# yjh0410/YOLO-Nano

Measured on AMD Instinct MI355X. Metric: images/sec YOLO-Nano-1.0x 416x416 bs=32 inference (network + decode + NMS + host delivery), higher is better.
Workload: dtype f32 (split-f16 MFMA x3, fp32 accumulate); 1 GPU; YOLO-Nano-1.0x 416x416 bs=32/GPU fp32 inference, COCO 80-class head + NMS (BASELINE configs[1]); inputs resident in HBM, kept detections delivered to pinned host memory inside the timed region; global_batch=32, parallelism=image-sharded x1, no collective, rccl_ranks=1, launch_mode=eager, streams_per_gpu=4

## Files before the change

yolo-nano_amd/csrc/kernels_post.hip:

```cpp
#include "yn_device.h"
#include "yn_head_tile_map.h"
#include "yn_prep.h"

namespace ynk {

__device__ __forceinline__ float sigmoid_f(float v) { return 1.0f / (1.0f + expf(-v)); }
__device__ __forceinline__ float exp_le0(float x) { return __builtin_amdgcn_exp2f(x * 1.44269504088896340736f); }

__device__ __forceinline__ void cand_location(const GridInfo& g, int n, int& s, int& cell, int& a)
{
    s = (n >= g.off[2]) ? 2 : ((n >= g.off[1]) ? 1 : 0);
    const int local = n - g.off[s];
    cell = local / g.A;
    a = local - cell * g.A;
}

__device__ __forceinline__ float grid_window_norm(const GridInfo& g, float p, int k)
{
    return (p + (float)((k & 1) ? g.top : g.left)) / (float)g.side;
}

__device__ __forceinline__ void decode_one(const GridInfo& g, int s, int cell, int a, const float* t, float S, float* box, bool normalise)
{
    const int gy = cell / g.w[s], gx = cell - gy * g.w[s];
// ... 1700 lines not shown
    const int n = seg_count[(size_t)b * C + c];
    const int T = (n + 63) >> 6;
    const bool sliced = rank < sliced_ranks && T - 1 > YN_PRE_W;
    const int ZS = sliced ? min(YN_PRE_Z, (T - 1 + YN_PRE_W - 1) / YN_PRE_W) : 1;
    bool decide = false;
    if (sliced && seg_sparse && sweep_slots > 0 && large_list && nms_colmajor(n)) {
        const int32_t* ll = large_list + (size_t)b * (large_cap + 1);
        const int nl = ll[0] < sweep_slots ? ll[0] : sweep_slots;
        for (int k = 0; k < nl; ++k) decide |= ll[1 + k] == c;
    }
    const bool decider = decide && z == ZS;
    if (z >= ZS && !decider) return;
    if (n == 0) { if (threadIdx.x == 0) { seg_count2[(size_t)b * C + c] = 0; if (seg_sparse) seg_sparse[(size_t)b * C + c] = 0; } return; }
    const int off = seg_off[(size_t)b * C + c];
    const float4* sb = sbox + (size_t)b * N + off;
    const int32_t* ids = bucket + (size_t)b * N + off;
    const int tid = threadIdx.x, lane = tid & 63;
    const int wave = __builtin_amdgcn_readfirstlane((int)(tid >> 6));
    const size_t slot = (size_t)b * YN_PRE_RANKS + (rank < YN_PRE_RANKS ? rank : 0);
    u64* ticket = pre_sync + slot;
    u64* gs = pre_sync + YN_PRE_TICKETS + slot * pre_sync_words(N);
    if (decider) {
        const bool sp = sweep_spread_out(sb, n, L);
        if (tid == 0) __hip_atomic_store(&gs[0], sp ? 1ull : 0ull, __ATOMIC_RELAXED, __HIP_MEMORY_SCOPE_AGENT);
    } else {
        float4* cbox = L.cbox[wave];
        float* carea = L.carea[wave];
        float4 bx0 = make_float4(0.f, 0.f, 0.f, 0.f);
        if (lane < n) bx0 = sb[lane];
        {
            u64 part = 0;
            if (wave * 8 < n) part = tile_word_boxes<false>(bx0, bx0, n, 0, 0, thresh, cbox, carea, wave * 8, wave * 8 + 8);
            L.dpart[lane][wave] = (unsigned char)(part >> (8 * wave));
        }
        __syncthreads();
        if (wave == 0) {
            const u64 diag = *reinterpret_cast<const u64*>(L.dpart[lane]);
            const int cnt = min(64, n);
            u64 alive = cnt == 64 ? ~0ull : ((1ull << cnt) - 1ull);
            u64 work = __ballot(((alive >> lane) & 1ull) && (diag & alive));
            const unsigned dlo = (unsigned)(diag & 0xffffffffu), dhi = (unsigned)(diag >> 32);
            while (work) {
                const int i = __ffsll((long long)work) - 1;
                const unsigned lo_i = (unsigned)__builtin_amdgcn_readlane((int)dlo, i);
                const unsigned hi_i = (unsigned)__builtin_amdgcn_readlane((int)dhi, i);
                alive &= ~(((u64)hi_i << 32) | (u64)lo_i);
                work &= alive & ~(1ull << i);
            }
            if (((alive >> lane) & 1ull) && z == 0) keep[(size_t)b * N + ids[lane]] = 1;
            if (lane == 0) L.keepm = alive;
        }
        if (T == 1) {
            if (tid == 0) { seg_count2[(size_t)b * C + c] = 0; if (seg_sparse) seg_sparse[(size_t)b * C + c] = 0; }
            return;
        }
        __syncthreads();
        const u64 keepm = L.keepm;
        const float4 bx = bx0;
        float4 cb = make_float4(0.f, 0.f, 0.f, 0.f), cbn = cb;
        int ci = 1 + z * YN_PRE_W + wave;
        if (ci < T && ci * 64 + lane < n) cb = sb[ci * 64 + lane];
        for (; ci < T; ci += YN_PRE_W * ZS) {
            const int cn = ci + YN_PRE_W * ZS;
            cbn = make_float4(0.f, 0.f, 0.f, 0.f);
            if (cn < T && cn * 64 + lane < n) cbn = sb[cn * 64 + lane];
            u64 w = keepm ? tile_word_boxes<false>(bx, cb, n, 0, ci, thresh, cbox, carea) : 0ull;
            w = ((keepm >> lane) & 1ull) ? w : 0ull;
            unsigned lo = (unsigned)(w & 0xffffffffu), hi = (unsigned)(w >> 32);
#pragma unroll
            for (int o = 32; o >= 1; o >>= 1) { lo |= __shfl_xor(lo, o); hi |= __shfl_xor(hi, o); }
            const int cnt = min(64, n - ci * 64);
            const u64 valid = cnt == 64 ? ~0ull : ((1ull << cnt) - 1ull);
            const u64 sv = valid & ~(((u64)hi << 32) | (u64)lo);
            if (lane == 0) { if (sliced) __hip_atomic_store(&gs[ci], sv, __ATOMIC_RELAXED, __HIP_MEMORY_SCOPE_AGENT); else L.surv[ci] = sv; }
            cb = cbn;
        }
    }
    bool spread = false;
    if (sliced) {
        asm volatile("s_waitcnt vmcnt(0)" ::: "memory");
        __syncthreads();
        if (tid == 0) {
            const u64 t = __hip_atomic_fetch_add(ticket, 1ull, __ATOMIC_RELAXED, __HIP_MEMORY_SCOPE_AGENT);
            L.last = t == (u64)(ZS + (decide ? 1 : 0) - 1);
            if (L.last) __hip_atomic_store(ticket, 0ull, __ATOMIC_RELAXED, __HIP_MEMORY_SCOPE_AGENT);
        }
        __syncthreads();
        if (!L.last) return;
        for (int k = 1 + tid; k < T; k += NTH) L.surv[k] = __hip_atomic_load(&gs[k], __ATOMIC_RELAXED, __HIP_MEMORY_SCOPE_AGENT);
        if (decide) spread = __hip_atomic_load(&gs[0], __ATOMIC_RELAXED, __HIP_MEMORY_SCOPE_AGENT) != 0ull;
    }
    __syncthreads();
    const int Q = (T - 1 + NTH - 1) / NTH;
    int mine = 0;
    for (int q = 0; q < Q; ++q) { const int ci = 1 + tid * Q + q; if (ci < T) mine += __popcll(L.surv[ci]); }
    L.part[tid] = mine;
    __syncthreads();
    for (int o = 1; o < NTH; o <<= 1) {
        const int v = tid >= o ? L.part[tid - o] : 0;
        __syncthreads();
        L.part[tid] += v;
        __syncthreads();
    }
    int run = L.part[tid] - mine;
    for (int q = 0; q < Q; ++q) { const int ci = 1 + tid * Q + q; if (ci < T) { L.base[ci] = run; run += __popcll(L.surv[ci]); } }
    const int n2 = L.part[NTH - 1];
    if (tid == NTH - 1) {
        seg_count2[(size_t)b * C + c] = n2;
        if (seg_sparse) seg_sparse[(size_t)b * C + c] = (spread && nms_colmajor(n2) && n2 <= sweep_maxn) ? 1 : 0;
    }
    __syncthreads();
    for (int ci = 1 + wave; ci < T; ci += YN_PRE_W) {
        const u64 m = L.surv[ci];
        if ((m >> lane) & 1ull) {
            const int dst = L.base[ci] + __popcll(m & ((1ull << lane) - 1ull));
            sbox2[(size_t)b * N + off + dst] = sb[ci * 64 + lane];
            bucket2[(size_t)b * N + off + dst] = ids[ci * 64 + lane];
        }
    }
}

__global__ __launch_bounds__(1024) void nms_sweep_kernel(const float4* __restrict__ sbox, const int32_t* __restrict__ seg_count, const int32_t* __restrict__ seg_off,
                                                         const int32_t* __restrict__ tile_off, int N, int C, float thresh, u64* __restrict__ M, size_t m_stride,
                                                         const int32_t* __restrict__ large_list, int large_cap, const int32_t* __restrict__ seg_sparse, int maxn)
{
    extern __shared__ __attribute__((aligned(16))) float4 sw_box[];
    __shared__ int start[YN_SWEEP_BINS + 2];
    __shared__ int irr[YN_SWEEP_IRR];
    __shared__ int wide[YN_SWEEP_WIDE];
    __shared__ int n_wide;
    __shared__ unsigned xlo_u, xhi_u;
    __shared__ int n_irr;
    const int b = blockIdx.x;
    const int32_t* ll = large_list + (size_t)b * (large_cap + 1);
    if ((int)blockIdx.z >= ll[0]) return;
    const int c = ll[1 + blockIdx.z];
    const int n = seg_count[(size_t)b * C + c];
    if (!nms_colmajor(n) || n > maxn || !seg_sparse[(size_t)b * C + c]) return;
    const float4* sb = sbox + (size_t)b * N + seg_off[(size_t)b * C + c];
    int* sw_order = reinterpret_cast<int*>(sw_box + n);
    const int tid = threadIdx.x, lane = tid & 63, wave = tid >> 6;
    for (int i = tid; i < YN_SWEEP_BINS + 2; i += 1024) start[i] = 0;
    if (tid == 0) { xlo_u = 0xffffffffu; xhi_u = 0u; n_irr = 0; n_wide = 0; }
    __syncthreads();
    {
        unsigned mn = 0xffffffffu, mx = 0u;
        for (int i = tid; i < n; i += 1024) {
            const float4 bx = sb[i];
            sw_box[i] = bx;
            if (sweep_regular(bx)) { mn = min(mn, order_bits(bx.x)); mx = max(mx, order_bits(bx.z)); }
            else { const int k = atomicAdd(&n_irr, 1); if (k < YN_SWEEP_IRR) irr[k] = i; }
        }
#pragma unroll
        for (int o = 32; o >= 1; o >>= 1) { mn = min(mn, (unsigned)__shfl_xor((int)mn, o)); mx = max(mx, (unsigned)__shfl_xor((int)mx, o)); }
        if (lane == 0) { atomicMin(&xlo_u, mn); atomicMax(&xhi_u, mx); }
    }
    __syncthreads();
    const int nirr = n_irr;
    const SweepBins bins(xlo_u, xhi_u);
    auto bin_of = [&](float x) { return bins.of(x); };
    for (int i = tid; i < n; i += 1024) {
        const float4 bx = sw_box[i];
        if (sweep_regular(bx)) atomicAdd(&start[bin_of(bx.x) + 2], 1);
    }
    __syncthreads();
    if (wave == 0) {
        int mine = 0;
        for (int q = 0; q < YN_SWEEP_BINS / 64; ++q) mine += start[2 + lane * (YN_SWEEP_BINS / 64) + q];
        int incl = mine;
#pragma unroll
        for (int o = 1; o < 64; o <<= 1) { const int v = __shfl_up(incl, o); if (lane >= o) incl += v; }
        int run = incl - mine;
        for (int q = 0; q < YN_SWEEP_BINS / 64; ++q) { const int k = 2 + lane * (YN_SWEEP_BINS / 64) + q; const int cnt = start[k]; start[k] = run; run += cnt; }
    }
    __syncthreads();
    for (int i = tid; i < n; i += 1024) {
        const float4 bx = sw_box[i];
        if (sweep_regular(bx)) sw_order[atomicAdd(&start[bin_of(bx.x) + 2], 1)] = i;
    }
    __syncthreads();
    u64* Ms = M + (size_t)b * m_stride + (size_t)tile_off[(size_t)b * (C + 1) + c] * 64;
    const float c_hi = thresh * 1.00001f, c_lo = thresh * 0.99999f;
    auto test = [&](int i, int j, const float4 bi, float ai, const float4 bj) {
        const float aj = (bj.z - bj.x) * (bj.w - bj.y);
        const float w = vmax_raw(1e-28f, vmin_raw(bi.z, bj.z) - vmax_raw(bi.x, bj.x));
        const float h = vmax_raw(1e-28f, vmin_raw(bi.w, bj.w) - vmax_raw(bi.y, bj.y));
        const float inter = w * h;
        const float un = (ai + aj) - inter;
        const float hi = un * c_hi, lo = un * c_lo;
        bool hit;
        if (lo > 1e-30f && inter < lo) return;
        if (lo > 1e-30f && inter > hi) hit = true;
        else hit = suppressed(bi, ai, bj, aj, thresh, 0);
        if (hit) {
            const int r = i < j ? i : j, t = i < j ? j : i;
            atomicOr(Ms + ctile_off(r >> 6, t >> 6) + (r & 63), 1ull << (t & 63));
        }
    };
    const int kz = blockIdx.y, KZ = gridDim.y;
    const int grp = tid >> 4, gl = tid & 15;
    for (int i = kz + KZ * grp; i < n; i += 64 * KZ) {
        const float4 bi = sw_box[i];
        if (!sweep_regular(bi)) continue;
        const float ai = (bi.z - bi.x) * (bi.w - bi.y);
        const int q0 = bin_of(bi.x), q1 = bin_of(bi.z);
        const int p0 = start[q0 + 1], pm = start[q0 + 2], p1 = start[q1 + 2];
        if (p1 - p0 > YN_SWEEP_WIDE_VISITS) {
            int k = 0;
            if (gl == 0) k = atomicAdd(&n_wide, 1);
            k = __shfl(k, 0, 16);
            if (k < YN_SWEEP_WIDE) { if (gl == 0) wide[k] = i; continue; }
        }
        for (int p = p0 + gl; p < p1; p += 16) {
            const int j = sw_order[p];
            if (p < pm ? j > i : true) test(i, j, bi, ai, sw_box[j]);
        }
    }
    __syncthreads();
    {
        const int nw = n_wide < YN_SWEEP_WIDE ? n_wide : YN_SWEEP_WIDE;
        for (int k = 0; k < nw; ++k) {
            const int i = wide[k];
            const float4 bi = sw_box[i];
            const float ai = (bi.z - bi.x) * (bi.w - bi.y);
            const int q0 = bin_of(bi.x), q1 = bin_of(bi.z);
            const int p0 = start[q0 + 1], pm = start[q0 + 2], p1 = start[q1 + 2];
            for (int p = p0 + tid; p < p1; p += 1024) {
                const int j = sw_order[p];
                if (p < pm ? j > i : true) test(i, j, bi, ai, sw_box[j]);
            }
        }
    }
    for (int k = 0; k < nirr; ++k) {
        const int i = irr[k];
        const float4 bi = sw_box[i];
        const float ai = (bi.z - bi.x) * (bi.w - bi.y);
        for (int j = kz + KZ * tid; j < n; j += 1024 * KZ) {
            if (j == i) continue;
            const float4 bj = sw_box[j];
            if (sweep_regular(bj) || j > i) test(i, j, bi, ai, bj);
        }
    }
}

__global__ __launch_bounds__(64) void nms_tile_off_kernel(const int32_t* __restrict__ seg_count2, int C, int32_t* __restrict__ tile_off2, const int32_t* __restrict__ seg_sparse,
                                                          int32_t* __restrict__ work_off)
{
    const int b = blockIdx.x, lane = threadIdx.x;
    int tiles = 0, wtiles = 0;
    for (int c0 = 0; c0 < C; c0 += 64) {
        const int c = c0 + lane;
        int t = 0, w = 0;
        if (c < C) {
            const int T = (seg_count2[(size_t)b * C + c] + 63) >> 6;
            t = T * (T + 1) / 2;
            w = (seg_sparse && seg_sparse[(size_t)b * C + c]) ? 0 : t;
        }
        int ti = t, wi = w;
#pragma unroll
        for (int o = 1; o < 64; o <<= 1) { const int a = __shfl_up(ti, o), d = __shfl_up(wi, o); if (lane >= o) { ti += a; wi += d; } }
        if (c < C) {
            tile_off2[(size_t)b * (C + 1) + c] = tiles + ti - t;
            if (work_off) work_off[(size_t)b * (C + 1) + c] = wtiles + wi - w;
        }
        tiles += __shfl(ti, 63);
        wtiles += __shfl(wi, 63);
    }
    if (lane == 0) {
        tile_off2[(size_t)b * (C + 1) + C] = tiles;
        if (work_off) work_off[(size_t)b * (C + 1) + C] = wtiles;
    }
}

__global__ __launch_bounds__(1024) void single_sort_kernel(const float* __restrict__ dets, const float* __restrict__ scores, int n,
                                                           int32_t* __restrict__ ids, float4* __restrict__ sbox, u64* __restrict__ gscratch)
{
    extern __shared__ __attribute__((aligned(16))) unsigned char sort_lds[];
    if (gscratch) sort_segment<false>(dets, scores, ids, false, n, nms_pow2(n), gscratch, sbox);
    else sort_segment<true>(dets, scores, ids, false, n, nms_pow2(n), reinterpret_cast<u64*>(sort_lds), sbox);
}

template <bool DIOU>
__global__ __launch_bounds__(64) void single_matrix_kernel(const float4* __restrict__ sbox, int n, float thresh, u64* __restrict__ M)
{
    __shared__ float4 cbox[64];
    __shared__ float carea[64];
    const int T = (n + 63) >> 6;
    const int total = T * (T + 1) / 2;
    for (int t = blockIdx.x; t < total; t += gridDim.x) {
        int rem = t, ri = 0;
        while (rem >= T - ri) { rem -= T - ri; ++ri; }
        matrix_tile<DIOU>(sbox, n, T, ri, ri + rem, thresh, M, cbox, carea);
    }
}

__global__ __launch_bounds__(256) void single_resolve_kernel(const int32_t* __restrict__ ids, int n, const u64* __restrict__ M,
                                                              int32_t* __restrict__ pick_list, int32_t* __restrict__ count)
{
    __shared__ ResolveLds L;
    const int picked = n > 0 ? resolve_segment<2>(ids, n, M, nullptr, pick_list, L) : 0;
    if (threadIdx.x == 0) *count = picked;
}

__global__ __launch_bounds__(1024) void compact_kernel(const float* __restrict__ boxes, const float* __restrict__ scores,
                                                        const int32_t* __restrict__ cls, const int32_t* __restrict__ keep, int N,
                                                        float* __restrict__ out_boxes, float* __restrict__ out_scores,
                                                        int32_t* __restrict__ out_cls, int32_t* __restrict__ out_index,
                                                        int32_t* __restrict__ count, const unsigned* __restrict__ ovf, unsigned* __restrict__ ovf_host)
{
    constexpr int IT = 32;
    __shared__ int wave_sums[IT][16];
    __shared__ int part[8];
    __shared__ int base, total_next;
    const int b = blockIdx.x;
    const int lane = threadIdx.x & 63, wave = threadIdx.x >> 6;
    if (threadIdx.x == 0) base = 0;
    __syncthreads();
    for (int n0 = 0; n0 < N; n0 += IT * 1024) {
        int kf[IT];
#pragma unroll
        for (int it = 0; it < IT; ++it) {
            const int n = n0 + it * 1024 + threadIdx.x;
            kf[it] = keep[(size_t)b * N + (n < N ? n : N - 1)];
        }
        unsigned flags = 0;
        int before[IT];
#pragma unroll
        for (int it = 0; it < IT; ++it) {
            const int n = n0 + it * 1024 + threadIdx.x;
            const int f = (n < N && kf[it]) ? 1 : 0;
            const unsigned long long bal = __ballot(f);
            before[it] = __popcll(bal & ((1ull << lane) - 1ull));
            if (lane == 0) wave_sums[it][wave] = __popcll(bal);
            flags |= (unsigned)f << it;
        }
        __syncthreads();
        int v = 0, incl = 0;
        if (threadIdx.x < IT * 16) {
            v = (&wave_sums[0][0])[threadIdx.x];
            incl = v;
#pragma unroll
            for (int o = 1; o < 64; o <<= 1) { const int t2 = __shfl_up(incl, o); if (lane >= o) incl += t2; }
            if (lane == 63) part[wave] = incl;
        }
        __syncthreads();
        if (threadIdx.x < IT * 16) {
            int add = 0;
#pragma unroll
            for (int w = 0; w < 8; ++w) add += (w < wave) ? part[w] : 0;
            (&wave_sums[0][0])[threadIdx.x] = base + add + incl - v;
            if (threadIdx.x == IT * 16 - 1) total_next = base + add + incl;
        }
        __syncthreads();
#pragma unroll
        for (int g8 = 0; g8 < IT; g8 += 8) {
            float4 bx[8]; float sc[8]; int cl[8];
#pragma unroll
            for (int k = 0; k < 8; ++k) {
                const int it = g8 + k;
                const int n = n0 + it * 1024 + threadIdx.x;
                const size_t src = (size_t)b * N + (((flags >> it) & 1u) ? n : 0);
                bx[k] = *reinterpret_cast<const float4*>(boxes + src * 4);
                sc[k] = scores[src];
                cl[k] = cls[src];
            }
#pragma unroll
            for (int k = 0; k < 8; ++k) {
                const int it = g8 + k;
                if ((flags >> it) & 1u) {
                    const int n = n0 + it * 1024 + threadIdx.x;
                    const size_t dst = (size_t)b * N + wave_sums[it][wave] + before[it];
                    *reinterpret_cast<float4*>(out_boxes + dst * 4) = bx[k];
                    out_scores[dst] = sc[k];
                    out_cls[dst] = cl[k];
                    if (out_index) out_index[dst] = n;
                }
            }
        }
        __syncthreads();
        if (threadIdx.x == 0) base = total_next;
        __syncthreads();
    }
    if (threadIdx.x == 0) {
        const bool flagged = ovf && *ovf;
        count[b] = flagged ? -1 - base : base;
        if (flagged && ovf_host) __hip_atomic_store(ovf_host, 1u, __ATOMIC_RELAXED, __HIP_MEMORY_SCOPE_SYSTEM);
    }
}

int nms_max_segment() { return 64 * YN_RESOLVE_MAX_T; }

__global__ __launch_bounds__(256) void pack_kernel(const float* __restrict__ boxes, const float* __restrict__ scores, const int32_t* __restrict__ cls,
                                                   const int32_t* __restrict__ count, int B, int N, float* __restrict__ rec, int32_t* __restrict__ offsets)
{
    __shared__ int base_s, total_s;
    const int b = blockIdx.x;
    if (threadIdx.x < 64) {
        int mine = 0, all = 0;
        int bad = 0;
        for (int i = threadIdx.x; i < B; i += 64) { int c = count[i]; if (c < 0) { bad = 1; c = -1 - c; } all += c; if (i < b) mine += c; }
        for (int o = 32; o > 0; o >>= 1) { mine += __shfl_xor(mine, o); all += __shfl_xor(all, o); bad |= __shfl_xor(bad, o); }
        if (threadIdx.x == 0) { base_s = mine; total_s = bad ? -1 - all : all; }
    }
    __syncthreads();
    const int base = base_s, k = count[b] < 0 ? -1 - count[b] : count[b];
    if (threadIdx.x == 0) { offsets[b] = base; if (b == 0) offsets[B] = total_s; }
    for (int i = threadIdx.x; i < k; i += 256) {
        const size_t src = (size_t)b * N + i;
        const float4 bx = *reinterpret_cast<const float4*>(boxes + src * 4);
        float* r = rec + (size_t)(base + i) * 6;
        *reinterpret_cast<float2*>(r) = make_float2(bx.x, bx.y);
        *reinterpret_cast<float2*>(r + 2) = make_float2(bx.z, bx.w);
        *reinterpret_cast<float2*>(r + 4) = make_float2(scores[src], (float)cls[src]);
    }
}

void launch_pack(const float* boxes, const float* scores, const int32_t* cls, const int32_t* count, int B, int N, float* rec, int32_t* offsets, hipStream_t s)
{
    hipLaunchKernelGGL(pack_kernel, dim3(B), dim3(256), 0, s, boxes, scores, cls, count, B, N, rec, offsets);
}

size_t nms_pre_sync_words(int B, int N) { return YN_PRE_TICKETS + (size_t)B * YN_PRE_RANKS * pre_sync_words(N); }
size_t nms_matrix_words_per_image(int N, int C)
{
    const size_t Tsum = (size_t)(N + 63) / 64 + C;
    return 64 * (Tsum * (Tsum + 1) / 2);
}

static void set_sort_attr()
{
    static unsigned long long done = 0;
    if (!attr_pending(done)) return;
    (void)hipFuncSetAttribute(reinterpret_cast<const void*>(sort_kernel), hipFuncAttributeMaxDynamicSharedMemorySize, YN_SORT_LARGE * 8);
    (void)hipFuncSetAttribute(reinterpret_cast<const void*>(single_sort_kernel), hipFuncAttributeMaxDynamicSharedMemorySize, YN_SORT_LARGE * 8);
}

const int32_t* launch_nms_bucket_sort(const float* boxes, const float* scores, const int32_t* cls, int B, int N, int C, const NmsWork& wk,
                                      hipStream_t s, const NmsHook* hook, NmsPlan& rec)
{
    set_sort_attr();
    const int large_cap = wk.large_cap;
    auto mark = [&](const char* k) { if (hook && hook->fn) hook->fn(hook->ctx, k); };
    float4* sbox = reinterpret_cast<float4*>(wk.sbox);
    u64* M = reinterpret_cast<u64*>(wk.matrix);
    constexpr int few_n = 16384;
    const bool few = (long)B * C <= 256 && N <= few_n;
    const int32_t* seg_order = wk.seg_order;
    rec.few = few;
    if (few && wk.ctr) {
        seg_order = nullptr;
        rec.fused = 1;
        static unsigned long long attr_bs = 0;
        if (attr_pending(attr_bs)) (void)hipFuncSetAttribute(reinterpret_cast<const void*>(bucket_sort_kernel), hipFuncAttributeMaxDynamicSharedMemorySize, YN_SORT_LARGE * 8);
        mark("bucket_sort_kernel");
        hipLaunchKernelGGL(bucket_sort_kernel, dim3(C, B), dim3(1024), YN_SORT_LARGE * 8, s, boxes, scores, cls, N, C, wk.seg_count, wk.seg_off, wk.tile_off, wk.bucket,
                           wk.keep, sbox, M, wk.matrix_stride, wk.ctr);
    } else {
        mark("bucket_kernel");
        hipLaunchKernelGGL(bucket_kernel, dim3(B), dim3(1024), 2 * C * sizeof(int32_t), s, cls, N, C, wk.seg_count, wk.seg_off, wk.tile_off, wk.bucket, wk.keep,
                           wk.large_list, large_cap, YN_SORT_SMALL, wk.seg_order);
        const bool chunks = !few && wk.large_list && (size_t)N <= wk.matrix_stride;
        rec.chunks = chunks;
        mark(chunks ? "sort_chunk_kernel" : "sort_kernel");
        if (few) {
            hipLaunchKernelGGL(sort_kernel, dim3(B, C), dim3(1024), YN_SORT_LARGE * 8, s, boxes, scores, wk.seg_count, wk.seg_off, wk.bucket, sbox,
                               N, C, 0, YN_SORT_LARGE, (u64*)nullptr, (size_t)0, (const int32_t*)nullptr, 0, (const int32_t*)wk.seg_order);
        } else if (chunks) {
            const int slots = N > YN_SORT_SMALL ? nms_chunk_slots(N, large_cap) : 0;
            hipLaunchKernelGGL(sort_chunk_kernel, dim3(B, C + slots), dim3(256), YN_SORT_SMALL * 8, s, boxes, scores, wk.seg_count, wk.seg_off, wk.bucket, sbox,
                               N, C, (const int32_t*)wk.seg_order, (const int32_t*)wk.large_list, large_cap, M, wk.matrix_stride);
            if (N > YN_SORT_SMALL) {
                mark("sort_merge_kernel");
                rec.merge = 1;
                hipLaunchKernelGGL(sort_merge_kernel, dim3((N + 255) / 256, B), dim3(256), 0, s, boxes, wk.seg_count, wk.seg_off, wk.bucket, sbox,
                                   N, C, (const int32_t*)wk.large_list, large_cap, (const u64*)M, wk.matrix_stride);
            }
        } else {
            hipLaunchKernelGGL(sort_kernel, dim3(B, C), dim3(256), YN_SORT_SMALL * 8, s, boxes, scores, wk.seg_count, wk.seg_off, wk.bucket, sbox,
                               N, C, 0, YN_SORT_SMALL, (u64*)nullptr, (size_t)0, (const int32_t*)nullptr, 0, (const int32_t*)wk.seg_order);
            if (N > YN_SORT_SMALL)
                hipLaunchKernelGGL(sort_kernel, dim3(large_cap, B), dim3(1024), YN_SORT_LARGE * 8, s, boxes, scores, wk.seg_count, wk.seg_off, wk.bucket, sbox,
                                   N, C, YN_SORT_SMALL, YN_SORT_LARGE, (u64*)nullptr, (size_t)0, (const int32_t*)wk.large_list, large_cap, (const int32_t*)nullptr);
        }
        if (N > YN_SORT_LARGE && !chunks)
            hipLaunchKernelGGL(sort_kernel, dim3(large_cap, B), dim3(1024), 0, s, boxes, scores, wk.seg_count, wk.seg_off, wk.bucket, sbox,
                               N, C, YN_SORT_LARGE, 1 << 30, M, wk.matrix_stride, (const int32_t*)wk.large_list, large_cap, (const int32_t*)nullptr);
    }
    return seg_order;
}

void launch_nms_compact(const float* boxes, const float* scores, const int32_t* cls, int B, int N, const NmsWork& wk,
                        float* out_boxes, float* out_scores, int32_t* out_cls, int32_t* out_index, int32_t* count, hipStream_t s)
{
    hipLaunchKernelGGL(compact_kernel, dim3(B), dim3(1024), 0, s, boxes, scores, cls, wk.keep, N, out_boxes, out_scores, out_cls, out_index, count, wk.ovf, wk.ovf_host);
}

void launch_nms_pipeline(const float* boxes, const float* scores, const int32_t* cls, int B, int N, int C,
                         float nms_thresh, int diou, const NmsWork& wk,
                         float* out_boxes, float* out_scores, int32_t* out_cls, int32_t* out_index, int32_t* count,
                         hipStream_t s, const NmsHook* hook, NmsPlan* plan)
{
    NmsPlan rec{};
    rec.B = B; rec.N = N; rec.C = C; rec.diou = diou != 0;
    const int large_cap = wk.large_cap;
    auto mark = [&](const char* k) { if (hook && hook->fn) hook->fn(hook->ctx, k); };
    float4* sbox = reinterpret_cast<float4*>(wk.sbox);
    u64* M = reinterpret_cast<u64*>(wk.matrix);
    const int32_t* seg_order = launch_nms_bucket_sort(boxes, scores, cls, B, N, C, wk, s, hook, rec);
    const bool few = rec.few != 0;
    const int32_t* m_count = wk.seg_count;
    const int32_t* m_toff = wk.tile_off;
    const int32_t* m_ids = wk.bucket;
    const float4* m_box = sbox;
    const int prefilter_env = wk.prefilter;
    bool sweep = false;
    int sweep_maxn = 0, sweep_slots = 0;
    if (!diou && wk.sbox2 && (prefilter_env == 2 || (prefilter_env == 1 && B >= 4))) {
        mark("nms_prefilter_kernel");
        sweep = wk.sweep && !few && wk.seg_sparse && wk.work_off && wk.large_list && large_cap > 0 && N > YN_SORT_SMALL && nms_thresh >= 1e-6f;
        sweep_maxn = N <= 16384 ? YN_SWEEP_MAXN / 2 : YN_SWEEP_MAXN;
        sweep_slots = large_cap < 4 ? large_cap : 4;
        const int pre_ranks = (seg_order && wk.pre_sync && (size_t)B * YN_PRE_RANKS <= YN_PRE_TICKETS) ? (C < YN_PRE_RANKS ? C : YN_PRE_RANKS) : 0;
        hipLaunchKernelGGL(nms_prefilter_kernel, dim3(B, C + pre_ranks * YN_PRE_Z), dim3(64 * YN_PRE_W), 0, s, sbox, wk.seg_count, wk.seg_off, wk.bucket, N, C, nms_thresh, wk.keep,
                           reinterpret_cast<float4*>(wk.sbox2), wk.bucket2, wk.seg_count2, seg_order, wk.seg_sparse, reinterpret_cast<u64*>(wk.pre_sync), pre_ranks,
                           (const int32_t*)wk.large_list, large_cap, sweep ? sweep_slots : 0, sweep_maxn);
        rec.prefilter = 1; rec.pre_ranks = pre_ranks;
        m_count = wk.seg_count2; m_toff = wk.tile_off2; m_ids = wk.bucket2; m_box = reinterpret_cast<const float4*>(wk.sbox2);
        mark("nms_tile_off_kernel");
        hipLaunchKernelGGL(nms_tile_off_kernel, dim3(B), dim3(64), 0, s, wk.seg_count2, C, wk.tile_off2, (const int32_t*)(sweep ? wk.seg_sparse : nullptr), sweep ? wk.work_off : nullptr);
    }
    int G = 4096 / (B > 0 ? B : 1);
    if (G < 32) G = 32;
    if (G > 2048) G = 2048;
    mark(diou ? "matrix_kernel<true>" : "matrix_kernel<false>");
    if (diou) hipLaunchKernelGGL(matrix_kernel<true>, dim3(G, B), dim3(256), 0, s, m_box, m_count, wk.seg_off, m_toff, N, C, nms_thresh, M, wk.matrix_stride,
                                 (const int32_t*)nullptr, (const int32_t*)nullptr, (const int32_t*)nullptr, 0);
    else      hipLaunchKernelGGL(matrix_kernel<false>, dim3(G, B), dim3(256), 0, s, m_box, m_count, wk.seg_off, m_toff, N, C, nms_thresh, M, wk.matrix_stride,
                                 (const int32_t*)(sweep ? wk.work_off : nullptr), (const int32_t*)(sweep ? wk.seg_sparse : nullptr), (const int32_t*)wk.large_list, large_cap);
    if (sweep) {
        mark("nms_sweep_kernel");
        int sweep_split = (sweep_maxn * 20 <= 64 * 1024 ? 256 : 128) / (B > 0 ? B : 1);
        sweep_split = sweep_split < 2 ? 2 : (sweep_split > 8 ? 8 : sweep_split);
        rec.sweep = 1; rec.sweep_maxn = sweep_maxn; rec.sweep_slots = sweep_slots; rec.sweep_split = sweep_split;
        static unsigned long long attr_sw = 0;
        if (attr_pending(attr_sw)) (void)hipFuncSetAttribute(reinterpret_cast<const void*>(nms_sweep_kernel), hipFuncAttributeMaxDynamicSharedMemorySize, YN_SWEEP_MAXN * 20);
        hipLaunchKernelGGL(nms_sweep_kernel, dim3(B, sweep_split, sweep_slots), dim3(1024), (size_t)sweep_maxn * 20, s, m_box, m_count, wk.seg_off, m_toff, N, C, nms_thresh,
                           M, wk.matrix_stride, (const int32_t*)wk.large_list, large_cap, (const int32_t*)wk.seg_sparse, sweep_maxn);
    }
    mark("resolve_kernel");
    const bool split = N > YN_SORT_SMALL && wk.large_list && large_cap > 0;
    rec.resolve_one = (long)B * C <= 256;
    rec.resolve_split = !rec.resolve_one && split;
    if ((long)B * C <= 256) {
        hipLaunchKernelGGL(resolve_large_kernel, dim3(C, B), dim3(512), 0, s, m_count, wk.seg_off, m_toff, m_ids, N, C, M, wk.matrix_stride,
                           wk.keep, (const int32_t*)nullptr, 0, 0);
    } else {
        hipLaunchKernelGGL(resolve_kernel, dim3(B, C), dim3(256), 0, s, m_count, wk.seg_off, m_toff, m_ids, N, C, M, wk.matrix_stride, wk.keep,
                           split ? YN_SORT_SMALL : 1 << 30, seg_order);
        if (split) hipLaunchKernelGGL(resolve_large_kernel, dim3(B, large_cap), dim3(512), 0, s, m_count, wk.seg_off, m_toff, m_ids, N, C, M, wk.matrix_stride,
                                      wk.keep, (const int32_t*)wk.large_list, large_cap, YN_SORT_SMALL);
    }
    mark("compact_kernel");
    hipLaunchKernelGGL(compact_kernel, dim3(B), dim3(1024), 0, s, boxes, scores, cls, wk.keep, N, out_boxes, out_scores, out_cls, out_index, count, wk.ovf, wk.ovf_host);
    if (plan) *plan = rec;
}

void launch_nms_single(const float* dets, const float* scores, int n, float thresh, int diou,
                       int32_t* ids_scratch, float* sbox_scratch, void* matrix_scratch, int32_t* keep, int32_t* count, hipStream_t s)
{
    set_sort_attr();
    float4* sbox = reinterpret_cast<float4*>(sbox_scratch);
    u64* M = reinterpret_cast<u64*>(matrix_scratch);
    if (n > 0) {
        const int P = nms_pow2(n);
        const int thr = P >= 2048 ? 1024 : 256;
        if (P <= YN_SORT_LARGE) hipLaunchKernelGGL(single_sort_kernel, dim3(1), dim3(thr), (size_t)P * 8, s, dets, scores, n, ids_scratch, sbox, (u64*)nullptr);
        else hipLaunchKernelGGL(single_sort_kernel, dim3(1), dim3(1024), 0, s, dets, scores, n, ids_scratch, sbox, M);
        const int T = (n + 63) / 64;
        int G = T * (T + 1) / 2;
        if (G > 8192) G = 8192;
        if (diou) hipLaunchKernelGGL(single_matrix_kernel<true>, dim3(G), dim3(64), 0, s, sbox, n, thresh, M);
        else      hipLaunchKernelGGL(single_matrix_kernel<false>, dim3(G), dim3(64), 0, s, sbox, n, thresh, M);
    }
    hipLaunchKernelGGL(single_resolve_kernel, dim3(1), dim3(256), 0, s, ids_scratch, n, M, keep, count);
}

__device__ __forceinline__ void preprocess_pixel(const PrepArgs& a, int i)
{
    if (i >= a.side * a.side) return;
    const int y = i / a.side, x = i - y * a.side;
    preprocess_at(a, y - a.top, x - a.left, (size_t)a.side * a.side, i);
}

__global__ __launch_bounds__(256) void preprocess_kernel(PrepArgs a) { preprocess_pixel(a, blockIdx.x * 256 + threadIdx.x); }

constexpr int PREP_MAX = 32;
struct PrepImg { const unsigned char* img; int h0, w0, rw, rh, left, top; };
struct PrepBatchArgs { PrepImg im[PREP_MAX]; int side; float mean[3], std[3]; float* out; };
__global__ __launch_bounds__(256) void preprocess_batch_kernel(PrepBatchArgs b)
{
    const PrepImg& d = b.im[blockIdx.y];
    PrepArgs a;
    a.img = d.img; a.h0 = d.h0; a.w0 = d.w0; a.pitch = d.w0; a.rw = d.rw; a.rh = d.rh; a.left = d.left; a.top = d.top; a.side = b.side;
    a.mode = prep_mode(d.h0, d.w0, d.rw, d.rh);
#pragma unroll
    for (int c = 0; c < 3; ++c) { a.mean[c] = b.mean[c]; a.std[c] = b.std[c]; }
    a.out = b.out + (size_t)blockIdx.y * 3 * b.side * b.side;
    preprocess_pixel(a, blockIdx.x * 256 + threadIdx.x);
}

struct PrepRectArgs { PrepImg im[PREP_MAX]; int win_left, win_top, win_w, win_h; float mean[3], std[3]; float* out; };
__global__ __launch_bounds__(256) void preprocess_batch_rect_kernel(PrepRectArgs b)
{
    const PrepImg& d = b.im[blockIdx.y];
    PrepArgs a;
    a.img = d.img; a.h0 = d.h0; a.w0 = d.w0; a.pitch = d.w0; a.rw = d.rw; a.rh = d.rh; a.left = d.left; a.top = d.top; a.side = 0;
    a.mode = prep_mode(d.h0, d.w0, d.rw, d.rh);
#pragma unroll
    for (int c = 0; c < 3; ++c) { a.mean[c] = b.mean[c]; a.std[c] = b.std[c]; }
    const size_t plane = (size_t)b.win_w * b.win_h;
    a.out = b.out + (size_t)blockIdx.y * 3 * plane;
    const int i = blockIdx.x * 256 + threadIdx.x;
    if (i >= b.win_w * b.win_h) return;
    const int y = i / b.win_w, x = i - y * b.win_w;
    preprocess_at(a, y + b.win_top - a.top, x + b.win_left - a.left, plane, i);
}

void launch_preprocess_batch_rect(int n, const unsigned char* const* imgs, const int* geom, int win_left, int win_top, int win_w, int win_h,
                                  const float* mean, const float* stdv, float* out, hipStream_t s)
{
    const size_t plane = (size_t)win_w * win_h;
    for (int i0 = 0; i0 < n; i0 += PREP_MAX) {
        const int m = n - i0 < PREP_MAX ? n - i0 : PREP_MAX;
        PrepRectArgs b{};
        for (int i = 0; i < m; ++i) {
            const int* g = geom + (size_t)(i0 + i) * 6;
            b.im[i] = PrepImg{imgs[i0 + i], g[0], g[1], g[2], g[3], g[4], g[5]};
        }
        b.win_left = win_left; b.win_top = win_top; b.win_w = win_w; b.win_h = win_h; b.out = out + (size_t)i0 * 3 * plane;
        for (int c = 0; c < 3; ++c) { b.mean[c] = mean[c]; b.std[c] = stdv[c]; }
        hipLaunchKernelGGL(preprocess_batch_rect_kernel, dim3((unsigned)((plane + 255) / 256), m), dim3(256), 0, s, b);
    }
}

void launch_preprocess_batch(int n, const unsigned char* const* imgs, const int* geom, int side, const float* mean, const float* stdv,
                             float* out, hipStream_t s)
{
    for (int i0 = 0; i0 < n; i0 += PREP_MAX) {
        const int m = n - i0 < PREP_MAX ? n - i0 : PREP_MAX;
        PrepBatchArgs b{};
        for (int i = 0; i < m; ++i) {
            const int* g = geom + (size_t)(i0 + i) * 6;
            b.im[i] = PrepImg{imgs[i0 + i], g[0], g[1], g[2], g[3], g[4], g[5]};
        }
        b.side = side; b.out = out + (size_t)i0 * 3 * side * side;
        for (int c = 0; c < 3; ++c) { b.mean[c] = mean[c]; b.std[c] = stdv[c]; }
        hipLaunchKernelGGL(preprocess_batch_kernel, dim3((side * side + 255) / 256, m), dim3(256), 0, s, b);
    }
}

void launch_preprocess(const unsigned char* img, int h0, int w0, int rw, int rh, int left, int top, int side,
                       const float* mean, const float* stdv, float* out, hipStream_t s)
{
    PrepArgs a;
    a.img = img; a.h0 = h0; a.w0 = w0; a.pitch = w0; a.rw = rw; a.rh = rh; a.left = left; a.top = top; a.side = side; a.out = out;
    for (int c = 0; c < 3; ++c) { a.mean[c] = mean[c]; a.std[c] = stdv[c]; }
    a.mode = prep_mode(h0, w0, rw, rh);
    const int n = side * side;
    hipLaunchKernelGGL(preprocess_kernel, dim3((n + 255) / 256), dim3(256), 0, s, a);
}

}
```

Baseline: 53710 images/s.

## Split compact and pack kernels across chunks per image

Compact now launches a 2D grid of 256-thread blocks, one per 1024-element chunk per image, instead of one 1024-thread block per image looping over all candidates. Each block recomputes its output offset by recounting keep flags of all earlier chunks with ballots, so the serial per-image loop disappears at the cost of redundant prefix counting that grows with position. Pack is similarly split into parts per image, each recomputing the cross-image base. With B=32 the old launches used only 32 blocks, so spreading the work should fill more compute units.

```diff
diff --git a/yolo-nano_amd/csrc/kernels_post.hip b/yolo-nano_amd/csrc/kernels_post.hip
--- a/yolo-nano_amd/csrc/kernels_post.hip
+++ b/yolo-nano_amd/csrc/kernels_post.hip
@@ -2026,122 +2026,143 @@
     if (threadIdx.x == 0) *count = picked;
 }
 
-__global__ __launch_bounds__(1024) void compact_kernel(const float* __restrict__ boxes, const float* __restrict__ scores,
-                                                        const int32_t* __restrict__ cls, const int32_t* __restrict__ keep, int N,
-                                                        float* __restrict__ out_boxes, float* __restrict__ out_scores,
-                                                        int32_t* __restrict__ out_cls, int32_t* __restrict__ out_index,
-                                                        int32_t* __restrict__ count, const unsigned* __restrict__ ovf, unsigned* __restrict__ ovf_host)
-{
-    constexpr int IT = 32;
-    __shared__ int wave_sums[IT][16];
-    __shared__ int part[8];
-    __shared__ int base, total_next;
-    const int b = blockIdx.x;
+constexpr int YN_COMPACT_IT = 4;
+constexpr int YN_COMPACT_CHUNK = 256 * YN_COMPACT_IT;
+static_assert(YN_COMPACT_CHUNK % 1024 == 0, "compact_kernel counts the earlier chunks in runs of 1 024 flags");
+struct __attribute__((packed, aligned(4))) Keep4 { int32_t x, y, z, w; };
+__global__ __launch_bounds__(256) void compact_kernel(const float* __restrict__ boxes, const float* __restrict__ scores,
+                                                       const int32_t* __restrict__ cls, const int32_t* __restrict__ keep, int N,
+                                                       float* __restrict__ out_boxes, float* __restrict__ out_scores,
+                                                       int32_t* __restrict__ out_cls, int32_t* __restrict__ out_index,
+                                                       int32_t* __restrict__ count, const unsigned* __restrict__ ovf, unsigned* __restrict__ ovf_host)
+{
+    constexpr int IT = YN_COMPACT_IT;
+    __shared__ int wave_sums[IT][4];
+    __shared__ int earlier_s[4];
+    const int b = blockIdx.y, c0 = blockIdx.x * YN_COMPACT_CHUNK;
     const int lane = threadIdx.x & 63, wave = threadIdx.x >> 6;
-    if (threadIdx.x == 0) base = 0;
-    __syncthreads();
-    for (int n0 = 0; n0 < N; n0 += IT * 1024) {
-        int kf[IT];
-#pragma unroll
-        for (int it = 0; it < IT; ++it) {
-            const int n = n0 + it * 1024 + threadIdx.x;
-            kf[it] = keep[(size_t)b * N + (n < N ? n : N - 1)];
-        }
-        unsigned flags = 0;
-        int before[IT];
-#pragma unroll
-        for (int it = 0; it < IT; ++it) {
-            const int n = n0 + it * 1024 + threadIdx.x;
-            const int f = (n < N && kf[it]) ? 1 : 0;
-            const unsigned long long bal = __ballot(f);
-            before[it] = __popcll(bal & ((1ull << lane) - 1ull));
-            if (lane == 0) wave_sums[it][wave] = __popcll(bal);
-            flags |= (unsigned)f << it;
-        }
-        __syncthreads();
-        int v = 0, incl = 0;
-        if (threadIdx.x < IT * 16) {
-            v = (&wave_sums[0][0])[threadIdx.x];
-            incl = v;
-#pragma unroll
-            for (int o = 1; o < 64; o <<= 1) { const int t2 = __shfl_up(incl, o); if (lane >= o) incl += t2; }
-            if (lane == 63) part[wave] = incl;
-        }
-        __syncthreads();
-        if (threadIdx.x < IT * 16) {
-            int add = 0;
-#pragma unroll
-            for (int w = 0; w < 8; ++w) add += (w < wave) ? part[w] : 0;
-            (&wave_sums[0][0])[threadIdx.x] = base + add + incl - v;
-            if (threadIdx.x == IT * 16 - 1) total_next = base + add + incl;
-        }
-        __syncthreads();
-#pragma unroll
-        for (int g8 = 0; g8 < IT; g8 += 8) {
-            float4 bx[8]; float sc[8]; int cl[8];
-#pragma unroll
-            for (int k = 0; k < 8; ++k) {
-                const int it = g8 + k;
-                const int n = n0 + it * 1024 + threadIdx.x;
-                const size_t src = (size_t)b * N + (((flags >> it) & 1u) ? n : 0);
-                bx[k] = *reinterpret_cast<const float4*>(boxes + src * 4);
-                sc[k] = scores[src];
-                cl[k] = cls[src];
-            }
-#pragma unroll
-            for (int k = 0; k < 8; ++k) {
-                const int it = g8 + k;
-                if ((flags >> it) & 1u) {
-                    const int n = n0 + it * 1024 + threadIdx.x;
-                    const size_t dst = (size_t)b * N + wave_sums[it][wave] + before[it];
-                    *reinterpret_cast<float4*>(out_boxes + dst * 4) = bx[k];
-                    out_scores[dst] = sc[k];
-                    out_cls[dst] = cl[k];
-                    if (out_index) out_index[dst] = n;
-                }
-            }
-        }
-        __syncthreads();
-        if (threadIdx.x == 0) base = total_next;
-        __syncthreads();
-    }
-    if (threadIdx.x == 0) {
+    const int32_t* kb = keep + (size_t)b * N;
+    if (N <= 0) {
+        if (threadIdx.x == 0) count[b] = (ovf && *ovf) ? -1 : 0;
+        return;
+    }
+    int kf[IT];
+#pragma unroll
+    for (int it = 0; it < IT; ++it) {
+        const int n = c0 + it * 256 + threadIdx.x;
+        kf[it] = kb[n < N ? n : N - 1];
+    }
+    int earlier = 0;
+    const int runs = c0 >> 10;
+    for (int r0 = 0; r0 < runs; r0 += 8) {
+        Keep4 v[8];
+#pragma unroll
+        for (int j = 0; j < 8; ++j) {
+            const int r = r0 + j < runs ? r0 + j : runs - 1;
+            v[j] = *reinterpret_cast<const Keep4*>(kb + (size_t)r * 1024 + threadIdx.x * 4);
+        }
+#pragma unroll
+        for (int j = 0; j < 8; ++j) {
+            const int c = __popcll(__ballot(v[j].x != 0)) + __popcll(__ballot(v[j].y != 0)) + __popcll(__ballot(v[j].z != 0)) + __popcll(__ballot(v[j].w != 0));
+            earlier += r0 + j < runs ? c : 0;
+        }
+    }
+    unsigned flags = 0;
+    int before[IT];
+#pragma unroll
+    for (int it = 0; it < IT; ++it) {
+        const int n = c0 + it * 256 + threadIdx.x;
+        const int f = (n < N && kf[it]) ? 1 : 0;
+        const unsigned long long bal = __ballot(f);
+        before[it] = __popcll(bal & ((1ull << lane) - 1ull));
+        if (lane == 0) wave_sums[it][wave] = __popcll(bal);
+        flags |= (unsigned)f << it;
+    }
+    if (lane == 0) earlier_s[wave] = earlier;
+    __syncthreads();
+    int pos = earlier_s[0] + earlier_s[1] + earlier_s[2] + earlier_s[3];
+    int first[IT];
+#pragma unroll
+    for (int it = 0; it < IT; ++it) {
+#pragma unroll
+        for (int w = 0; w < 4; ++w) {
+            if (w == wave) first[it] = pos;
+            pos += wave_sums[it][w];
+        }
+    }
+    float4 bx[IT]; float sc[IT]; int cl[IT];
+#pragma unroll
+    for (int it = 0; it < IT; ++it) {
+        const int n = c0 + it * 256 + threadIdx.x;
+        const size_t src = (size_t)b * N + (((flags >> it) & 1u) ? n : 0);
+        bx[it] = *reinterpret_cast<const float4*>(boxes + src * 4);
+        sc[it] = scores[src];
+        cl[it] = cls[src];
+    }
+#pragma unroll
+    for (int it = 0; it < IT; ++it)
+        asm volatile("" : "+v"(bx[it].x), "+v"(bx[it].y), "+v"(bx[it].z), "+v"(bx[it].w), "+v"(sc[it]), "+v"(cl[it]));
+#pragma unroll
+    for (int it = 0; it < IT; ++it) {
+        if ((flags >> it) & 1u) {
+            const int n = c0 + it * 256 + threadIdx.x;
+            const size_t dst = (size_t)b * N + first[it] + before[it];
+            *reinterpret_cast<float4*>(out_boxes + dst * 4) = bx[it];
+            out_scores[dst] = sc[it];
+            out_cls[dst] = cl[it];
+            if (out_index) out_index[dst] = n;
+        }
+    }
+    if (blockIdx.x == gridDim.x - 1 && threadIdx.x == 0) {
         const bool flagged = ovf && *ovf;
-        count[b] = flagged ? -1 - base : base;
+        count[b] = flagged ? -1 - pos : pos;
         if (flagged && ovf_host) __hip_atomic_store(ovf_host, 1u, __ATOMIC_RELAXED, __HIP_MEMORY_SCOPE_SYSTEM);
     }
 }
 
 int nms_max_segment() { return 64 * YN_RESOLVE_MAX_T; }
 
+constexpr int YN_PACK_ROWS = 4;
+constexpr int YN_PACK_PART = 256 * YN_PACK_ROWS;
 __global__ __launch_bounds__(256) void pack_kernel(const float* __restrict__ boxes, const float* __restrict__ scores, const int32_t* __restrict__ cls,
                                                    const int32_t* __restrict__ count, int B, int N, float* __restrict__ rec, int32_t* __restrict__ offsets)
 {
-    __shared__ int base_s, total_s;
-    const int b = blockIdx.x;
-    if (threadIdx.x < 64) {
-        int mine = 0, all = 0;
-        int bad = 0;
-        for (int i = threadIdx.x; i < B; i += 64) { int c = count[i]; if (c < 0) { bad = 1; c = -1 - c; } all += c; if (i < b) mine += c; }
-        for (int o = 32; o > 0; o >>= 1) { mine += __shfl_xor(mine, o); all += __shfl_xor(all, o); bad |= __shfl_xor(bad, o); }
-        if (threadIdx.x == 0) { base_s = mine; total_s = bad ? -1 - all : all; }
-    }
-    __syncthreads();
-    const int base = base_s, k = count[b] < 0 ? -1 - count[b] : count[b];
-    if (threadIdx.x == 0) { offsets[b] = base; if (b == 0) offsets[B] = total_s; }
-    for (int i = threadIdx.x; i < k; i += 256) {
-        const size_t src = (size_t)b * N + i;
-        const float4 bx = *reinterpret_cast<const float4*>(boxes + src * 4);
-        float* r = rec + (size_t)(base + i) * 6;
-        *reinterpret_cast<float2*>(r) = make_float2(bx.x, bx.y);
-        *reinterpret_cast<float2*>(r + 2) = make_float2(bx.z, bx.w);
-        *reinterpret_cast<float2*>(r + 4) = make_float2(scores[src], (float)cls[src]);
+    const int b = blockIdx.y, lane = threadIdx.x & 63;
+    const int cb = count[b], k = cb < 0 ? -1 - cb : cb;
+    const int i0 = blockIdx.x * YN_PACK_PART;
+    if (i0 >= k && blockIdx.x != 0) return;
+    int base = 0, all = 0, bad = 0;
+    for (int i = lane; i < B; i += 64) { int c = count[i]; if (c < 0) { bad = 1; c = -1 - c; } all += c; if (i < b) base += c; }
+    for (int o = 32; o > 0; o >>= 1) { base += __shfl_xor(base, o); all += __shfl_xor(all, o); bad |= __shfl_xor(bad, o); }
+    if (blockIdx.x == 0 && threadIdx.x == 0) { offsets[b] = base; if (b == 0) offsets[B] = bad ? -1 - all : all; }
+    if (i0 >= k) return;
+    float4 bx[YN_PACK_ROWS]; float sc[YN_PACK_ROWS]; int cl[YN_PACK_ROWS];
+#pragma unroll
+    for (int r = 0; r < YN_PACK_ROWS; ++r) {
+        const int i = i0 + r * 256 + threadIdx.x;
+        const size_t src = (size_t)b * N + (i < k ? i : 0);
+        bx[r] = *reinterpret_cast<const float4*>(boxes + src * 4);
+        sc[r] = scores[src];
+        cl[r] = cls[src];
+    }
+#pragma unroll
+    for (int r = 0; r < YN_PACK_ROWS; ++r) asm volatile("" : "+v"(bx[r].x), "+v"(bx[r].y), "+v"(bx[r].z), "+v"(bx[r].w));
+#pragma unroll
+    for (int r = 0; r < YN_PACK_ROWS; ++r) {
+        const int i = i0 + r * 256 + threadIdx.x;
+        if (i < k) {
+            float* q = rec + (size_t)(base + i) * 6;
+            *reinterpret_cast<float2*>(q) = make_float2(bx[r].x, bx[r].y);
+            *reinterpret_cast<float2*>(q + 2) = make_float2(bx[r].z, bx[r].w);
+            *reinterpret_cast<float2*>(q + 4) = make_float2(sc[r], (float)cl[r]);
+        }
     }
 }
 
 void launch_pack(const float* boxes, const float* scores, const int32_t* cls, const int32_t* count, int B, int N, float* rec, int32_t* offsets, hipStream_t s)
 {
-    hipLaunchKernelGGL(pack_kernel, dim3(B), dim3(256), 0, s, boxes, scores, cls, count, B, N, rec, offsets);
+    const int parts = N > 0 ? (N + YN_PACK_PART - 1) / YN_PACK_PART : 1;
+    hipLaunchKernelGGL(pack_kernel, dim3(parts, B), dim3(256), 0, s, boxes, scores, cls, count, B, N, rec, offsets);
 }
 
 size_t nms_pre_sync_words(int B, int N) { return YN_PRE_TICKETS + (size_t)B * YN_PRE_RANKS * pre_sync_words(N); }
@@ -2216,7 +2237,8 @@
 void launch_nms_compact(const float* boxes, const float* scores, const int32_t* cls, int B, int N, const NmsWork& wk,
                         float* out_boxes, float* out_scores, int32_t* out_cls, int32_t* out_index, int32_t* count, hipStream_t s)
 {
-    hipLaunchKernelGGL(compact_kernel, dim3(B), dim3(1024), 0, s, boxes, scores, cls, wk.keep, N, out_boxes, out_scores, out_cls, out_index, count, wk.ovf, wk.ovf_host);
+    const int chunks = N > 0 ? (N + YN_COMPACT_CHUNK - 1) / YN_COMPACT_CHUNK : 1;
+    hipLaunchKernelGGL(compact_kernel, dim3(chunks, B), dim3(256), 0, s, boxes, scores, cls, wk.keep, N, out_boxes, out_scores, out_cls, out_index, count, wk.ovf, wk.ovf_host);
 }
 
 void launch_nms_pipeline(const float* boxes, const float* scores, const int32_t* cls, int B, int N, int C,
@@ -2285,7 +2307,7 @@
                                       wk.keep, (const int32_t*)wk.large_list, large_cap, YN_SORT_SMALL);
     }
     mark("compact_kernel");
-    hipLaunchKernelGGL(compact_kernel, dim3(B), dim3(1024), 0, s, boxes, scores, cls, wk.keep, N, out_boxes, out_scores, out_cls, out_index, count, wk.ovf, wk.ovf_host);
+    launch_nms_compact(boxes, scores, cls, B, N, wk, out_boxes, out_scores, out_cls, out_index, count, s);
     if (plan) *plan = rec;
 }
 
```

Measured after the change: 54070 images/s (median of 6 runs). About the same (+0.7%).
